# aponte411/minGPT-distributed

Hardware: AMD Instinct MI355X
Metric: tokens/sec (whole node), GPT-2 124M seq1024 bf16 (higher is better)
Workload: dtype bf16; 1 GPU; model=gpt2, global_batch=128, seq_len=1024, parallelism=dp1, micro_batch_per_gpu=128, hip_graph=False

## Files before the change

### csrc/kernels/xent.hip

```cpp
#include "common.h"
#include "kernels.h"

using namespace mg;

namespace {

__global__ __launch_bounds__(256) void xent_fwd_kernel(const bf16_t* __restrict__ logits,
                                                       const int64_t* __restrict__ targets,
                                                       float* __restrict__ loss_row,
                                                       float* __restrict__ lse_out, int V, int ld,
                                                       unsigned int* __restrict__ err) {
  __shared__ float red[8];
  const long row = blockIdx.x;
  const bf16_t* lr = logits + row * ld;
  float mx = -INFINITY, sm = 0.f;
  const int V8 = V & ~7;
  for (int c = threadIdx.x * 8; c < V8; c += 256 * 8) {
    float v[8];
    unpack8(ld16(lr + c), v);
    float lm = v[0];
#pragma unroll
    for (int j = 1; j < 8; ++j) lm = fmaxf(lm, v[j]);
    if (lm > mx) {
      sm *= __expf(mx - lm);
      mx = lm;
    }
#pragma unroll
    for (int j = 0; j < 8; ++j) sm += __expf(v[j] - mx);
  }
  for (int c = V8 + threadIdx.x; c < V; c += 256) {
    const float v = bf2f(lr[c]);
    if (v > mx) {
      sm *= __expf(mx - v);
      mx = v;
    }
    sm += __expf(v - mx);
  }
  const float gmx = block_max<4>(mx, red);
  sm = (mx == -INFINITY) ? 0.f : sm * __expf(mx - gmx);
  const float gsm = block_sum<4>(sm, red + 4);
  if (threadIdx.x == 0) {
    const float lse = gmx + __logf(gsm);
    lse_out[row] = lse;
    long t = targets[row];
  MG_CHECK_INDEX(t, t < V, -1, err, 4u)
    loss_row[row] = (t < 0) ? 0.f : lse - bf2f(lr[t]);
  }
}

__global__ __launch_bounds__(1024) void xent_finalize_kernel(const float* __restrict__ loss_row,
                                                             const int64_t* __restrict__ targets,
                                                             float* __restrict__ out, int M) {
  __shared__ float red[32];
  float s = 0.f, n = 0.f;
  for (int i = threadIdx.x; i < M; i += 1024) {
    s += loss_row[i];
    n += targets[i] >= 0 ? 1.f : 0.f;
  }
  s = block_sum<16>(s, red);
  n = block_sum<16>(n, red + 16);
  if (threadIdx.x == 0) {
    const float inv = n > 0.f ? 1.f / n : 0.f;
    out[0] = s * inv;
    out[1] = inv;
  }
}

__global__ __launch_bounds__(256) void xent_bwd_kernel(const bf16_t* __restrict__ logits,
                                                       const int64_t* __restrict__ targets,
                                                       const float* __restrict__ lse,
                                                       const float* __restrict__ gscale,
                                                       const float* __restrict__ inv_n,
                                                       bf16_t* __restrict__ dlogits, int V, int ld,
                                                       unsigned int* __restrict__ err) {
  const long row = blockIdx.x;
  long t = targets[row];
  MG_CHECK_INDEX(t, t < V, -1, err, 4u)
  const float g = (t < 0) ? 0.f : gscale[0] * inv_n[0];
  const float l = lse[row];
  const bf16_t* lr = logits + row * ld;
  bf16_t* dr = dlogits + row * ld;
  for (int c = threadIdx.x * 8; c < ld; c += 256 * 8) {
    float v[8];
    if (c + 8 <= V) {
      unpack8(ld16(lr + c), v);
#pragma unroll
      for (int j = 0; j < 8; ++j) v[j] = g * (__expf(v[j] - l) - ((c + j) == t ? 1.f : 0.f));
    } else {
#pragma unroll
      for (int j = 0; j < 8; ++j) {
        const int cj = c + j;
        v[j] = cj < V ? g * (__expf(bf2f(lr[cj]) - l) - (cj == t ? 1.f : 0.f)) : 0.f;
      }
    }
    st16(dr + c, pack8(v));
  }
}


__global__ __launch_bounds__(1024) void xent_count_kernel(const int64_t* __restrict__ targets,
                                                          float* __restrict__ out, int M) {
  __shared__ float red[16];
  float n = 0.f;
  for (int i = threadIdx.x; i < M; i += 1024) n += targets[i] >= 0 ? 1.f : 0.f;
  n = block_sum<16>(n, red);
  if (threadIdx.x == 0) out[1] = n > 0.f ? 1.f / n : 0.f;
}

template <int NV>
__global__ __launch_bounds__(1024) void xent_fused_kernel(const bf16_t* __restrict__ logits,
                                                          const int64_t* __restrict__ targets,
                                                          const float* __restrict__ inv_n,
                                                          float* __restrict__ loss_row,
                                                          bf16_t* __restrict__ dlogits, int V,
                                                          int ld, unsigned int* __restrict__ err) {
  __shared__ float red[32];
  const long row = blockIdx.x;
  const bf16_t* lr = logits + row * ld;
  bf16_t* dr = dlogits + row * ld;
  constexpr uint32_t NEG2 = 0xFF80FF80u;
  uint4 u[NV];
#pragma unroll
  for (int k = 0; k < NV; ++k) {
    const int c = (threadIdx.x + k * 1024) * 8;
    if (c + 8 <= V) {
      u[k] = ld16_nt(lr + c);
    } else if (c < V) {
      float f[8];
#pragma unroll
      for (int j = 0; j < 8; ++j) f[j] = (c + j < V) ? bf2f(lr[c + j]) : -INFINITY;
      u[k] = pack8(f);
    } else {
      u[k] = make_uint4(NEG2, NEG2, NEG2, NEG2);
    }
  }
  float mx = -INFINITY;
#pragma unroll
  for (int k = 0; k < NV; ++k) {
    float v[8];
    unpack8(u[k], v);
#pragma unroll
    for (int j = 0; j < 8; ++j) mx = fmaxf(mx, v[j]);
  }
  const float gmx = block_max<16>(mx, red);
#pragma unroll
  for (int k = 0; k < NV; ++k) reg_fence(u[k]);
  constexpr float L2E = 1.4426950408889634f;
  const float mb = gmx * L2E;
  float sm = 0.f;
#pragma unroll
  for (int k = 0; k < NV; ++k) {
    float v[8];
    unpack8(u[k], v);
#pragma unroll
    for (int j = 0; j < 8; ++j) sm += exp2f(fmaf(v[j], L2E, -mb));
  }
  const float gsm = block_sum<16>(sm, red + 16);
#pragma unroll
  for (int k = 0; k < NV; ++k) reg_fence(u[k]);
  const float lse = gmx + __logf(gsm);
  long t = targets[row];
  MG_CHECK_INDEX(t, t < V, -1, err, 4u)
  const float g = (t < 0) ? 0.f : inv_n[0];
  const float lb = lse * L2E;
#pragma unroll
  for (int k = 0; k < NV; ++k) {
    const int c = (threadIdx.x + k * 1024) * 8;
    if (c < ld) {
      float v[8];
      unpack8(u[k], v);
#pragma unroll
      for (int j = 0; j < 8; ++j) v[j] = g * (exp2f(fmaf(v[j], L2E, -lb)) - ((c + j) == t ? 1.f : 0.f));
      st16_nt(dr + c, pack8(v));
    }
  }
  if (threadIdx.x == 0) loss_row[row] = (t < 0) ? 0.f : lse - bf2f(lr[t]);
}

__global__ __launch_bounds__(256) void xent_scale_kernel(bf16_t* __restrict__ dl,
                                                         const float* __restrict__ gscale, long n8) {
  const float s = gscale[0];
  if (s == 1.f) return;
  for (long i = blockIdx.x * 256L + threadIdx.x; i < n8; i += (long)gridDim.x * 256) {
    float v[8];
    unpack8(ld16(dl + i * 8), v);
#pragma unroll
    for (int j = 0; j < 8; ++j) v[j] *= s;
    st16(dl + i * 8, pack8(v));
  }
}

}

namespace mg {

void xent_fwd(const bf16_t* logits, const int64_t* targets, float* loss_row, float* lse, float* out,
              int M, int V, int ld, hipStream_t stream) {
  xent_fwd_kernel<<<M, 256, 0, stream>>>(logits, targets, loss_row, lse, V, ld, debug_err_word());
  xent_finalize_kernel<<<1, 1024, 0, stream>>>(loss_row, targets, out, M);
}

void xent_bwd(const bf16_t* logits, const int64_t* targets, const float* lse, const float* gscale,
              const float* inv_n, bf16_t* dlogits, int M, int V, int ld, hipStream_t stream) {
  xent_bwd_kernel<<<M, 256, 0, stream>>>(logits, targets, lse, gscale, inv_n, dlogits, V, ld, debug_err_word());
}

}

namespace mg {

int xent_fused_nv(int ld) {
  const int nv = (ld / 8 + 1023) / 1024;
  return (nv >= 4 && nv <= 8) ? nv : 0;
}

void xent_fused(const bf16_t* logits, const int64_t* targets, float* loss_row, float* out,
                bf16_t* dlogits, int M, int V, int ld, hipStream_t stream) {
  xent_count_kernel<<<1, 1024, 0, stream>>>(targets, out, M);
  switch (xent_fused_nv(ld)) {
#define MG_XF(n) \
  case n: xent_fused_kernel<n><<<M, 1024, 0, stream>>>(logits, targets, out + 1, loss_row, dlogits, V, ld, debug_err_word()); break;
    MG_XF(4) MG_XF(5) MG_XF(6) MG_XF(7) MG_XF(8)
#undef MG_XF
    default: break;
  }
  xent_finalize_kernel<<<1, 1024, 0, stream>>>(loss_row, targets, out, M);
}

void xent_scale(bf16_t* dlogits, const float* gscale, long n, hipStream_t stream) {
  const long n8 = n / 8;
  const long blocks = std::min<long>((n8 + 255) / 256, 2048);
  xent_scale_kernel<<<(int)blocks, 256, 0, stream>>>(dlogits, gscale, n8);
}

}
```

Measured before the change: 1.102 million tokens/s.

## Parallelize xent count, specialize tail handling, and use raw exp2/log in fused kernel

Replaces the single-block target count with a multi-block kernel that packs a count and a block-completion counter into one 64-bit atomic, preceded by a memset. The finalize kernel then skips recounting and reuses the stored inverse. The fused cross-entropy kernel gets a compile-time no-tail variant that drops bounds checks on leading chunks. It also uses the raw hardware exp2/log builtins and applies the one-hot subtraction only in the thread holding the target. The aim is to shorten the serial count/finalize launches and trim ALU work per logit, at the cost of an extra memset and atomic traffic.

Result: no change. 1.110 million tokens/s, median of 6 (+0.7%).

```diff
diff --git a/csrc/kernels/xent.hip b/csrc/kernels/xent.hip
--- a/csrc/kernels/xent.hip
+++ b/csrc/kernels/xent.hip
@@ -48,21 +48,35 @@
   }
 }
 
+constexpr int kFinGroup = 16;
+
+template <bool COUNT>
 __global__ __launch_bounds__(1024) void xent_finalize_kernel(const float* __restrict__ loss_row,
                                                              const int64_t* __restrict__ targets,
                                                              float* __restrict__ out, int M) {
   __shared__ float red[32];
   float s = 0.f, n = 0.f;
-  for (int i = threadIdx.x; i < M; i += 1024) {
-    s += loss_row[i];
-    n += targets[i] >= 0 ? 1.f : 0.f;
+  for (int i0 = threadIdx.x; i0 < M; i0 += kFinGroup * 1024) {
+    float l[kFinGroup];
+    bool valid[kFinGroup];
+#pragma unroll
+    for (int j = 0; j < kFinGroup; ++j) {
+      const int i = i0 + j * 1024;
+      l[j] = i < M ? loss_row[i] : 0.f;
+      if (COUNT) valid[j] = i < M && targets[i] >= 0;
+    }
+#pragma unroll
+    for (int j = 0; j < kFinGroup; ++j) {
+      if (i0 + j * 1024 < M) s += l[j];
+      if (COUNT) n += valid[j] ? 1.f : 0.f;
+    }
   }
   s = block_sum<16>(s, red);
-  n = block_sum<16>(n, red + 16);
+  if (COUNT) n = block_sum<16>(n, red + 16);
   if (threadIdx.x == 0) {
-    const float inv = n > 0.f ? 1.f / n : 0.f;
+    const float inv = COUNT ? (n > 0.f ? 1.f / n : 0.f) : out[1];
     out[0] = s * inv;
-    out[1] = inv;
+    if (COUNT) out[1] = inv;
   }
 }
 
@@ -98,16 +112,42 @@
 }
 
 
-__global__ __launch_bounds__(1024) void xent_count_kernel(const int64_t* __restrict__ targets,
-                                                          float* __restrict__ out, int M) {
-  __shared__ float red[16];
-  float n = 0.f;
-  for (int i = threadIdx.x; i < M; i += 1024) n += targets[i] >= 0 ? 1.f : 0.f;
-  n = block_sum<16>(n, red);
-  if (threadIdx.x == 0) out[1] = n > 0.f ? 1.f / n : 0.f;
-}
-
-template <int NV>
+constexpr int kCountRows = 1024;
+
+__global__ __launch_bounds__(256) void xent_count_kernel(const int64_t* __restrict__ targets,
+                                                         float* __restrict__ out, int M) {
+  __shared__ unsigned int red[4];
+  unsigned int n = 0;
+#pragma unroll
+  for (int j = 0; j < kCountRows / 256; ++j) {
+    const int i = blockIdx.x * kCountRows + j * 256 + threadIdx.x;
+    n += (i < M && targets[i] >= 0) ? 1u : 0u;
+  }
+#pragma unroll
+  for (int o = 32; o > 0; o >>= 1) n += __shfl_xor(n, o, 64);
+  if ((threadIdx.x & 63) == 0) red[threadIdx.x >> 6] = n;
+  __syncthreads();
+  if (threadIdx.x == 0) {
+    const unsigned long long mine = red[0] + red[1] + red[2] + red[3];
+    const unsigned long long old = atomicAdd(reinterpret_cast<unsigned long long*>(out), (mine << 32) | 1ull);
+    if ((unsigned int)old == gridDim.x - 1) {
+      const float nf = (float)(unsigned int)((old >> 32) + mine);
+      out[1] = nf > 0.f ? 1.f / nf : 0.f;
+    }
+  }
+}
+
+MG_DEVICE float exp2_le0(float x) { return __builtin_amdgcn_exp2f(x); }
+
+MG_DEVICE float log_normal(float x) {
+  constexpr float LN2_HI = 0x1.62e42ep-1f, LN2_LO = 0x1.efa39ep-25f;
+  const float y = __builtin_amdgcn_logf(x);
+  const float r = y * LN2_HI;
+  const float e = fmaf(y, LN2_LO, fmaf(y, LN2_HI, -r));
+  return fabsf(y) < INFINITY ? fmaf(LN2_HI, y, e) : y;
+}
+
+template <int NV, bool ANYTAIL>
 __global__ __launch_bounds__(1024) void xent_fused_kernel(const bf16_t* __restrict__ logits,
                                                           const int64_t* __restrict__ targets,
                                                           const float* __restrict__ inv_n,
@@ -119,11 +159,12 @@
   const bf16_t* lr = logits + row * ld;
   bf16_t* dr = dlogits + row * ld;
   constexpr uint32_t NEG2 = 0xFF80FF80u;
+  constexpr int KT = ANYTAIL ? 0 : NV - 1;
   uint4 u[NV];
 #pragma unroll
   for (int k = 0; k < NV; ++k) {
     const int c = (threadIdx.x + k * 1024) * 8;
-    if (c + 8 <= V) {
+    if (k < KT || c + 8 <= V) {
       u[k] = ld16_nt(lr + c);
     } else if (c < V) {
       float f[8];
@@ -153,24 +194,36 @@
     float v[8];
     unpack8(u[k], v);
 #pragma unroll
-    for (int j = 0; j < 8; ++j) sm += exp2f(fmaf(v[j], L2E, -mb));
+    for (int j = 0; j < 8; ++j) sm += exp2_le0(fmaf(v[j], L2E, -mb));
   }
   const float gsm = block_sum<16>(sm, red + 16);
 #pragma unroll
   for (int k = 0; k < NV; ++k) reg_fence(u[k]);
-  const float lse = gmx + __logf(gsm);
+  const float lse = gmx + log_normal(gsm);
   long t = targets[row];
   MG_CHECK_INDEX(t, t < V, -1, err, 4u)
   const float g = (t < 0) ? 0.f : inv_n[0];
   const float lb = lse * L2E;
-#pragma unroll
-  for (int k = 0; k < NV; ++k) {
-    const int c = (threadIdx.x + k * 1024) * 8;
-    if (c < ld) {
+  const int ti = t < 0 ? -1 : (int)t;
+  const int tv = ti >> 3;
+  uint32_t hot[8];
+#pragma unroll
+  for (int j = 0; j < 8; ++j) hot[j] = (ti & 7) == j ? 0x3f800000u : 0u;
+#pragma unroll
+  for (int k = 0; k < NV; ++k) {
+    const int vi = threadIdx.x + k * 1024, c = vi * 8;
+    if (k < NV - 1 || c < ld) {
       float v[8];
       unpack8(u[k], v);
 #pragma unroll
-      for (int j = 0; j < 8; ++j) v[j] = g * (exp2f(fmaf(v[j], L2E, -lb)) - ((c + j) == t ? 1.f : 0.f));
+      for (int j = 0; j < 8; ++j) v[j] = exp2_le0(fmaf(v[j], L2E, -lb));
+      if (vi == tv) {
+        asm volatile("; one-hot");
+#pragma unroll
+        for (int j = 0; j < 8; ++j) v[j] -= __uint_as_float(hot[j]);
+      }
+#pragma unroll
+      for (int j = 0; j < 8; ++j) v[j] *= g;
       st16_nt(dr + c, pack8(v));
     }
   }
@@ -197,7 +250,7 @@
 void xent_fwd(const bf16_t* logits, const int64_t* targets, float* loss_row, float* lse, float* out,
               int M, int V, int ld, hipStream_t stream) {
   xent_fwd_kernel<<<M, 256, 0, stream>>>(logits, targets, loss_row, lse, V, ld, debug_err_word());
-  xent_finalize_kernel<<<1, 1024, 0, stream>>>(loss_row, targets, out, M);
+  xent_finalize_kernel<true><<<1, 1024, 0, stream>>>(loss_row, targets, out, M);
 }
 
 void xent_bwd(const bf16_t* logits, const int64_t* targets, const float* lse, const float* gscale,
@@ -216,15 +269,23 @@
 
 void xent_fused(const bf16_t* logits, const int64_t* targets, float* loss_row, float* out,
                 bf16_t* dlogits, int M, int V, int ld, hipStream_t stream) {
-  xent_count_kernel<<<1, 1024, 0, stream>>>(targets, out, M);
-  switch (xent_fused_nv(ld)) {
-#define MG_XF(n) \
-  case n: xent_fused_kernel<n><<<M, 1024, 0, stream>>>(logits, targets, out + 1, loss_row, dlogits, V, ld, debug_err_word()); break;
+  (void)hipMemsetAsync(out, 0, 2 * sizeof(float), stream);
+  xent_count_kernel<<<std::max(1, cdiv(M, kCountRows)), 256, 0, stream>>>(targets, out, M);
+  const int nv = xent_fused_nv(ld);
+  const bool anytail = V < (nv - 1) * 8192;
+  switch (nv) {
+#define MG_XF(n)                                                                                                       \
+  case n:                                                                                                              \
+    if (anytail)                                                                                                       \
+      xent_fused_kernel<n, true><<<M, 1024, 0, stream>>>(logits, targets, out + 1, loss_row, dlogits, V, ld, debug_err_word()); \
+    else                                                                                                               \
+      xent_fused_kernel<n, false><<<M, 1024, 0, stream>>>(logits, targets, out + 1, loss_row, dlogits, V, ld, debug_err_word()); \
+    break;
     MG_XF(4) MG_XF(5) MG_XF(6) MG_XF(7) MG_XF(8)
 #undef MG_XF
     default: break;
   }
-  xent_finalize_kernel<<<1, 1024, 0, stream>>>(loss_row, targets, out, M);
+  xent_finalize_kernel<false><<<1, 1024, 0, stream>>>(loss_row, targets, out, M);
 }
 
 void xent_scale(bf16_t* dlogits, const float* gscale, long n, hipStream_t stream) {
```
